# Zhouxunzhe/ManiSkill

Hardware: AMD Instinct MI355X
Metric: env-steps/sec (whole node), PickCube-v1 state-obs 4096 envs/GPU (higher is better)
Workload: dtype f32; 1 GPU; PickCube-v1, Panda, state obs [N,42], pd_joint_delta_pos, num_envs=4096/GPU, sim 100 Hz / control 20 Hz = 5 substeps, 15+1 solver iterations, random actions 2*U-1, no resets inside the timed region; envs_per_gpu=4096, substeps=5, parallelism=env-sharded x1, no collective on the env path, solver_overflow_envs=0

## Files before the change

maniskill_amd/csrc/mssim_solve16.h:

```cpp
#pragma once
#include "mssim_limits.h"

#ifndef S16_WAVES
#define S16_WAVES 4
#endif
#define WSYNC() do { __builtin_amdgcn_fence(__ATOMIC_RELEASE, "wavefront"); __builtin_amdgcn_wave_barrier(); __builtin_amdgcn_fence(__ATOMIC_ACQUIRE, "wavefront"); } while (0)
#define BSYNC() __syncthreads()
#ifndef S16_ENVS_PER_BLOCK
#define S16_ENVS_PER_BLOCK 4
#endif
#define S16_COM_(nr) ((nr) == 4 ? 300 : 0)
#define S16_COM S16_COM_(NR)
#define S16_ANC 8
#define S16_VEC 32
#define S16_PT 96
#define S16_PT_LINK 1
#define S16_PT_FREE 17
#define S16_MAX_FREE S16_MAX_FREE_(NR)
#define S16_PT_KIN_(nr) (S16_PT_FREE + S16_MAX_FREE_(nr))
#define S16_PT_KIN S16_PT_KIN_(NR)
#define S16_MAX_HIT 64
#define S16_BP (S16_PT + 7 * S16_PT_LINK)
#define S16_U_(nr) ((nr) == 4 ? 320 : 272)
#define S16_U S16_U_(NR)
// ... 779 lines not shown
            float r[24];
            const float4* rp = reinterpret_cast<const float4*>(M.shape_pack + 24 * s);
#pragma unroll
            for (int k2 = 0; k2 < 6; k2++) { const float4 t = rp[k2]; r[4 * k2] = t.x; r[4 * k2 + 1] = t.y; r[4 * k2 + 2] = t.z; r[4 * k2 + 3] = t.w; }
            int ty = __float_as_int(r[18]);
            const int slot = __float_as_int(r[21]);
            int hull_first = M.shape_hull[2 * s], hull_count = M.shape_hull[2 * s + 1];
            if (slot < 0) {
              shF[k] = pose_t{f3{r[0], r[1], r[2]}, qnormalized(q4{r[3], r[4], r[5], r[6]})};
              shP[k][0] = r[7]; shP[k][1] = r[8]; shP[k][2] = r[9];
              shBc[k] = f3{r[10], r[11], r[12]};
              shBr[k] = r[13];
              shH[k] = f3{r[14], r[15], r[16]};
            } else {
              shF[k] = pose_soa(M.env_shape_frame, 7 * slot, N, e);
              const float* pp = M.env_shape_param + (size_t)(4 * slot) * N + e;
              const int w0 = __float_as_int(pp[0]);
              ty = w0 & 7;
              shP[k][0] = pp[(size_t)N]; shP[k][1] = pp[2 * (size_t)N]; shP[k][2] = pp[3 * (size_t)N];
              const float* bb = M.env_shape_bound + (size_t)(4 * slot) * N + e;
              shBc[k] = f3{bb[0], bb[(size_t)N], bb[2 * (size_t)N]};
              shBr[k] = bb[3 * (size_t)N];
              shH[k] = (ty == SH_BOX || ty == SH_CONVEX || ty == SH_TRIMESH) ? f3{shP[k][0], shP[k][1], shP[k][2]}
                     : ty == SH_SPHERE ? f3{shP[k][0], shP[k][0], shP[k][0]}
                     : ty == SH_CAPSULE ? f3{shP[k][1] + shP[k][0], shP[k][0], shP[k][0]}
                     : f3{shP[k][1], shP[k][0], shP[k][0]};
              hull_count = (w0 >> 3) & 127; hull_first = w0 >> 10;
            }
            shMu[k] = r[17];
            shTr[k] = r[22];
            shSlot[k] = pose_slot<NR>(__float_as_int(r[19]), __float_as_int(r[20]));
            shPk[k] = (unsigned)ty | ((unsigned)hull_count << 3) | ((unsigned)(shSlot[k] + 1) << 10) | ((unsigned)hull_first << 15);
          }
        }
      }
      EXP_DUP(DUP_SHAPE)
#pragma unroll
      for (int k = 0; k < 2; k++) {
        const int s = cl + GW * k;
        if (s < M.n_shape) {
          pose_t P = pose_t{f3{0, 0, 0}, q4{1, 0, 0, 0}};
          if (shSlot[k] >= 0) P = lds_pose(L + S16_PT + 7 * shSlot[k]);
          const pose_t W = pmul(P, shF[k]);
          const f3 bcw = P.p + qrot(P.q, shBc[k]);
          float* o = L + S16_NP_SHP + S16_SHP * s;
          lds_pose_store(o, W);
          o[7] = shP[k][0]; o[8] = shP[k][1]; o[9] = shP[k][2];
          o[10] = bcw.x; o[11] = bcw.y; o[12] = bcw.z; o[13] = shBr[k];
          o[14] = __uint_as_float(shPk[k]);
          o[15] = shMu[k];
          o[16] = shH[k].x; o[17] = shH[k].y; o[18] = shH[k].z; o[19] = shTr[k];
        }
      }
      WSYNC();
      PH(22);
      int nh = 0;
      int nmesh = 0;
      bool hit_over = false;
      auto cull_round = [&](int p, int sab) __attribute__((always_inline)) {
        bool surv = false;
        const int sa = sab & 0xFF, sb = (sab >> 8) & 0xFF;
        if (sab >= 0) {
          const float* ta_ = L + S16_NP_SHP + S16_SHP * sa;
          const float* tb_ = L + S16_NP_SHP + S16_SHP * sb;
          const int ta = (int)(__float_as_uint(ta_[14]) & 7u);
          const f3 cb = f3{tb_[10], tb_[11], tb_[12]};
          const float ra = ta_[13], rb = tb_[13];
          bool cull;
          if (ta == SH_PLANE) {
            const m3 R = qmat(q4{ta_[3], ta_[4], ta_[5], ta_[6]});
            cull = dot(mcol(R, 0), cb - f3{ta_[0], ta_[1], ta_[2]}) > rb + M.contact_offset;
          } else {
            const f3 d = cb - f3{ta_[10], ta_[11], ta_[12]};
            const float rr = ra + rb + M.contact_offset;
            cull = dot(d, d) > rr * rr;
          }
          const int s1a = (int)((__float_as_uint(ta_[14]) >> 10) & 31u), s1b = (int)((__float_as_uint(tb_[14]) >> 10) & 31u);
          auto inactive = [&](int s1) {
            const int b = s1 - 1 - S16_PT_FREE;
            return s1 == 0 || (b >= 0 && b < S16_MAX_FREE && fw_at(b) <= 0.f);
          };
          const int tb = (int)(__float_as_uint(tb_[14]) & 7u);
          surv = !cull && !(inactive(s1a) && inactive(s1b)) && ta != SH_NONE && tb != SH_NONE;
        }
        const unsigned long long bal = __ballot(surv);
        const unsigned m16 = (unsigned)(bal >> (16 * g)) & 0xFFFFu;
        if (surv) reinterpret_cast<int*>(L)[S16_NP_SCR + nh + __popc(m16 & ((1u << c) - 1u))] = p | (sa << 16) | (sb << 24);
        nh += __popc(m16);
      };
#ifdef EXP_CULL_ROUNDS
      const int n_pair_cull = M.n_pair < 16 * EXP_CULL_ROUNDS ? M.n_pair : 16 * EXP_CULL_ROUNDS;
#else
      const int n_pair_cull = M.n_pair;
#endif
      EXP_DUP(DUP_CULL) {
      if (dup_) { WSYNC(); nh = 0; nmesh = 0; }
      EXP_DUP(DUP_CULL1) {
        if (dup_) { WSYNC(); nh = 0; }
        int sab_next = lead ? M.pair_packed[c] : -1;
#pragma unroll 1
        for (int base = 0; base < n_pair_cull; base += 16) {
          const int sab = sab_next;
          sab_next = lead ? M.pair_packed[base + 16 + c] : -1;
          cull_round(base + c, sab);
        }
      }
      WSYNC();
      const int nh_s1 = nh;
      EXP_DUP(DUP_CULL2) {
        int nh2 = 0;
        if (dup_) { WSYNC(); nmesh = 0; }
#pragma unroll 1
        for (int base = 0; base < nh_s1; base += 16) {
          const int idx = base + c;
          bool keep = false, mesh = false;
          int pk = 0;
          if (idx < nh_s1) {
            pk = reinterpret_cast<const int*>(L)[S16_NP_SCR + idx];
            const float* ta_ = L + S16_NP_SHP + S16_SHP * ((pk >> 16) & 0xFF);
            const float* tb_ = L + S16_NP_SHP + S16_SHP * ((pk >> 24) & 0xFF);
            keep = true;
            if ((int)(__float_as_uint(ta_[14]) & 7u) != SH_PLANE) {
              const m3 RA = qmat(q4{ta_[3], ta_[4], ta_[5], ta_[6]}), RB = qmat(q4{tb_[3], tb_[4], tb_[5], tb_[6]});
              const f3 d = f3{tb_[10], tb_[11], tb_[12]} - f3{ta_[10], ta_[11], ta_[12]};
              keep = !obb_separated(RA, f3{ta_[16], ta_[17], ta_[18]}, RB, f3{tb_[16], tb_[17], tb_[18]}, d, M.contact_offset);
            }
            mesh = TRI && keep && (int)(__float_as_uint(tb_[14]) & 7u) == SH_TRIMESH;
            keep = keep && !mesh;
          }
          if (TRI) {
            const unsigned mm = (unsigned)(__ballot(mesh) >> (16 * g)) & 0xFFFFu;
            const int rankm = nmesh + __popc(mm & ((1u << c) - 1u));
            if (mesh) {
              if (rankm < S16_MAX_HIT) reinterpret_cast<int*>(L)[S16_REC + rankm] = pk;
              else hit_over = true;
            }
            nmesh = min(nmesh + __popc(mm), S16_MAX_HIT);
          }
          const unsigned m16 = (unsigned)(__ballot(keep) >> (16 * g)) & 0xFFFFu;
          const int rank = nh2 + __popc(m16 & ((1u << c) - 1u));
          if (keep) {
            if (rank < S16_MAX_HIT) reinterpret_cast<int*>(L)[S16_NP_HIT + rank] = pk;
            else hit_over = true;
          }
          nh2 += __popc(m16);
        }
        nh = nh2 < S16_MAX_HIT ? nh2 : S16_MAX_HIT;
        if (!live) { nh = 0; nmesh = 0; }
      }
      }
      WSYNC();
      if (__any(hit_over) && hit_over && live) atomicOr(&S.overflow[e], MSSIM_OVERFLOW_HITS);
      PH(23);
      int nml = 0;
      int nbl = 0;
      int npl = 0;
      {
        unsigned char* const ml = reinterpret_cast<unsigned char*>(L + S16_NP_ML);
        unsigned char* const bl = reinterpret_cast<unsigned char*>(L + S16_NP_BL);
        unsigned char* const pll = reinterpret_cast<unsigned char*>(L + S16_NP_PL);
        bool over = false;
        for (int base = 0; base < nh; base += 16) {
          const int idx = base + c;
          bool is_mpr = false, is_bb = false, is_ph = false;
          if (idx < nh) {
            const int pk = reinterpret_cast<const int*>(L)[S16_NP_HIT + idx];
            const int ta = (int)(__float_as_uint(L[S16_NP_SHP + S16_SHP * ((pk >> 16) & 0xFF) + 14]) & 7u);
            const int tb = (int)(__float_as_uint(L[S16_NP_SHP + S16_SHP * ((pk >> 24) & 0xFF) + 14]) & 7u);
            is_bb = ta == SH_BOX && tb == SH_BOX;
            is_ph = ta == SH_PLANE && tb == SH_CONVEX;
            is_mpr = !(ta == SH_PLANE || is_bb || (TRI && tb == SH_TRIMESH));
            reinterpret_cast<int*>(L)[S16_NP_CNT + idx] = 0;
          }
          const unsigned m16 = (unsigned)(__ballot(is_mpr) >> (16 * g)) & 0xFFFFu;
          const int rank = nml + __popc(m16 & ((1u << c) - 1u));
          if (is_mpr) {
            if (rank < S16_MAX_MPR) ml[rank] = (unsigned char)idx;
            else over = true;
          }
          nml += __popc(m16);
          const unsigned b16 = (unsigned)(__ballot(is_bb) >> (16 * g)) & 0xFFFFu;
          if (is_bb) bl[nbl + __popc(b16 & ((1u << c) - 1u))] = (unsigned char)idx;
          nbl += __popc(b16);
          const unsigned p16 = (unsigned)(__ballot(is_ph) >> (16 * g)) & 0xFFFFu;
          if (is_ph) pll[npl + __popc(p16 & ((1u << c) - 1u))] = (unsigned char)idx;
          npl += __popc(p16);
        }
        if (__any(over) && over && live) atomicOr(&S.overflow[e], MSSIM_OVERFLOW_CONVEX);
        nml = nml < S16_MAX_MPR ? nml : S16_MAX_MPR;
      }
      int cum[EPW + 1], mcum[EPW + 1], bcum[EPW + 1];
      cum[0] = mcum[0] = bcum[0] = 0;
#pragma unroll
      for (int j = 0; j < EPW; j++) {
        cum[j + 1] = cum[j] + __shfl(nh, GW * j);
        mcum[j + 1] = mcum[j] + __shfl(nml, GW * j);
        bcum[j + 1] = bcum[j] + __shfl(nbl, GW * j);
      }
      const int T = cum[EPW], TM = mcum[EPW], TB = bcum[EPW];
      const bool bb_lane = NR == 1 && TB > S16_MAX_BBC && T <= 64;
      bool pool_over = false;
      WSYNC();
      PH_ADD(14, (TM + EPW - 1) / EPW);
      (void)mcum;
      PH_ADD(26, T);
      auto pool_alloc = [&](float* Lg, int cnt) __attribute__((always_inline)) -> int {
        int off = atomicAdd(reinterpret_cast<int*>(Lg + S16_NP_ALLOC), cnt);
        if (off + cnt > MSSIM_MAX_RAW_POINTS) { pool_over = true; off = -1; }
        return off;
      };
      for (int t0 = 0; t0 < T; t0 += 64) {
        const int t = t0 + lane64;
        const bool has = t < T;
        int ge = 0;
#pragma unroll
        for (int j = 1; j < EPW; j++) ge += (has && t >= cum[j]) ? 1 : 0;
        const int idx = has ? t - cum[ge] : 0;
        float* Lg = smw + ge * S16_ENV_FLOATS;
        manifold_t m;
        manifold_clear(m);
        bool mine = false;
        if (has) {
          const int pk = reinterpret_cast<const int*>(Lg)[S16_NP_HIT + idx];
          const shape_t A = shape_from_table(M, Lg + S16_NP_SHP + S16_SHP * ((pk >> 16) & 0xFF));
          const shape_t B = shape_from_table(M, Lg + S16_NP_SHP + S16_SHP * ((pk >> 24) & 0xFF));
          PH_ADD(27, __popcll(__ballot(A.type == SH_PLANE)));
          PH_ADD(28, __popcll(__ballot(A.type == SH_BOX && B.type == SH_BOX)));
          PH(10);
          const bool is_plane = A.type == SH_PLANE && B.type != SH_CONVEX, is_bb = bb_lane && A.type == SH_BOX && B.type == SH_BOX;
          if (is_plane) collide_plane(A, B, M.contact_offset, m);
          PH(11);
          if (is_bb) collide_box_box<16>(A, B, M.contact_offset, m, L + S16_NP_SCR + c);
          PH(12);
          mine = is_plane || is_bb;
        }
        WSYNC();
        if (t0 == 0) {
          if (c == 0 && lead) reinterpret_cast<int*>(L)[S16_NP_ALLOC] = 0;
          WSYNC();
        }
        if (mine && m.count > 0) {
          const int off = pool_alloc(Lg, m.count);
          if (off >= 0) {
            reinterpret_cast<int*>(Lg)[S16_NP_CNT + idx] = m.count;
            reinterpret_cast<int*>(Lg)[S16_NP_OFF + idx] = off;
            float* hn = Lg + S16_NP_HN + 3 * idx;
            hn[0] = m.n.x; hn[1] = m.n.y; hn[2] = m.n.z;
#pragma unroll
            for (int k = 0; k < 4; k++)
              if (k < m.count) *reinterpret_cast<float4*>(Lg + S16_NP_POOL + 4 * (off + k)) = float4{m.x[k].x, m.x[k].y, m.x[k].z, m.sep[k]};
          }
        }
      }
      if (T == 0) {
        if (c == 0 && lead) reinterpret_cast<int*>(L)[S16_NP_ALLOC] = 0;
      }
      if (c == 0 && lead) { blk_nml[gb] = nml; blk_nbl[gb] = bb_lane ? 0 : nbl; blk_npl[gb] = npl; }
      BSYNC();
      PH(13);
      BT_T0b;
      {
        int4 hd = int4{-1, 0, 0, 0};
        if (live && nml > 0) hd = *reinterpret_cast<const int4*>(S.pcm + ((size_t)e * MSSIM_PCM_SLOTS + c) * S16_PCM_LEN);
        const int4 hd0 = hd;
        unsigned char* const slot_of = reinterpret_cast<unsigned char*>(L + S16_NP_SLOT);
        const unsigned char* const ml = reinterpret_cast<const unsigned char*>(L + S16_NP_ML);
        auto b16 = [&](bool v) __attribute__((always_inline)) { return (unsigned)(__ballot(v) >> (16 * g)) & 0xFFFFu; };
        for (int k = 0; k < nml; k++) {
          const int idx = ml[k];
          const int p = reinterpret_cast<const int*>(L)[S16_NP_HIT + idx] & 0xFFFF;
          unsigned m16 = b16(hd.x == p);
          bool fresh = false;
          if (m16 == 0u) {
            fresh = true;
            m16 = b16(hd.x < 0);
            if (m16 == 0u) {
              int st = hd.z < pcm_tick ? hd.z : 0x7FFFFFFF;
              int mn = st;
              mn = min(mn, __builtin_amdgcn_update_dpp(0, mn, 0x128, 0xF, 0xF, false));
              mn = min(mn, __builtin_amdgcn_update_dpp(0, mn, 0x124, 0xF, 0xF, false));
              mn = min(mn, __builtin_amdgcn_update_dpp(0, mn, 0x122, 0xF, 0xF, false));
              mn = min(mn, __builtin_amdgcn_update_dpp(0, mn, 0x121, 0xF, 0xF, false));
              m16 = mn != 0x7FFFFFFF ? b16(st == mn) : 0u;
            }
          }
          const int si = m16 ? (__ffs(m16) - 1) : -1;
          if (c == si) {
            if (fresh) { hd.x = p; hd.y = 0; hd.w = 0; }
            hd.z = pcm_tick;
          }
          if (c == 0) slot_of[idx] = si < 0 ? 255 : (unsigned char)(si | (fresh ? 0x80 : 0));
        }
        if (live && (hd.x != hd0.x || hd.y != hd0.y || hd.z != hd0.z || hd.w != hd0.w))
          *reinterpret_cast<int4*>(S.pcm + ((size_t)e * MSSIM_PCM_SLOTS + c) * S16_PCM_LEN) = hd;
      }
      __threadfence_block();
      BSYNC();
      BT_T(17);
      int TMb = 0;
#pragma unroll
      for (int j = 0; j < BLK_ENVS; j++) TMb += blk_nml[j];
      for (int t0 = 0; t0 < TMb; t0 += BLK_GRPS) {
        const bool has = t0 + grp < TMb;
        const int t = has ? t0 + grp : t0;
        int ge = 0, k = t;
#pragma unroll
        for (int j = 0; j < BLK_ENVS - 1; j++) {
          const int nj = blk_nml[j];
          const bool past = ge == j && k >= nj;
          k -= past ? nj : 0;
          ge += past ? 1 : 0;
        }
        float* Lg = sm + ge * S16_ENV_FLOATS;
        const int idx = reinterpret_cast<const unsigned char*>(Lg + S16_NP_ML)[k];
        const int pk = reinterpret_cast<const int*>(Lg)[S16_NP_HIT + idx];
        const shape_t A = shape_from_table(M, Lg + S16_NP_SHP + S16_SHP * ((pk >> 16) & 0xFF));
        const shape_t B = shape_from_table(M, Lg + S16_NP_SHP + S16_SHP * ((pk >> 24) & 0xFF));
        SupCoop16 sup;
        sup.c = c;
        SupCoop16::load_one(sup.va, A, c);
        SupCoop16::load_one(sup.vb, B, c);
        const int sbyte = reinterpret_cast<const unsigned char*>(Lg + S16_NP_SLOT)[idx];
        const bool cached = has && sbyte != 255;
        const bool fresh = cached && (sbyte & 0x80);
        float* const slot = S.pcm + ((size_t)(chunk * BLK_ENVS + ge) * MSSIM_PCM_SLOTS + (cached ? (sbyte & 15) : 0)) * S16_PCM_LEN;
        auto b16 = [&](bool v) __attribute__((always_inline)) { return (unsigned)(__ballot(v) >> (16 * g)) & 0xFFFFu; };
        int npts = 0, grow = 0;
        bool queried_empty = false;
        f3 relp0 = f3{0, 0, 0}, nloc = f3{1, 0, 0};
        float relR0[9] = {1, 0, 0, 0, 1, 0, 0, 0, 1};
        f3 pA = f3{0, 0, 0}, pB = f3{0, 0, 0};
        float s0 = 0.f;
        if (cached && !fresh) {
          const int4 h4 = *reinterpret_cast<const int4*>(slot);
          npts = h4.y; grow = h4.w >> 8; queried_empty = h4.w & 1;
          const float4 r1 = *reinterpret_cast<const float4*>(slot + 4), r2 = *reinterpret_cast<const float4*>(slot + 8), r3 = *reinterpret_cast<const float4*>(slot + 12),
                       r4 = *reinterpret_cast<const float4*>(slot + 16);
          relp0 = f3{r1.x, r1.y, r1.z};
          relR0[0] = r2.x; relR0[1] = r2.y; relR0[2] = r2.z; relR0[3] = r2.w; relR0[4] = r3.x; relR0[5] = r3.y; relR0[6] = r3.z; relR0[7] = r3.w; relR0[8] = r4.x;
          nloc = f3{r4.y, r4.z, r4.w};
          if (c < 4) {
            const float* pp = slot + 20 + 7 * c;
            pA = f3{pp[0], pp[1], pp[2]}; pB = f3{pp[3], pp[4], pp[5]}; s0 = pp[6];
          }
        }
        BT_T(18);
        const float offset = M.contact_offset;
        {
          const f3 nw = mmulv(A.rot, nloc);
          const f3 wA = A.c + mmulv(A.rot, pA), wB = B.c + mmulv(B.rot, pB);
          const f3 d = wA - wB;
          const float dn = dot(d, nw);
          const f3 tt = d - nw * dn;
// ... 472 lines not shown
            }
          } else if (A.type == SH_SPHERE) {
            cand1(0, A.c, A.p0, c == 0);
          } else if (A.type == SH_CAPSULE) {
            const f3 ax = mcol(A.rot, 0) * A.p1;
            cand1(0, c == 0 ? A.c - ax : A.c + ax, A.p0, c < 2);
          } else if (A.type == SH_CONVEX) {
#pragma unroll
            for (int k = 0; k < 4; k++) cand1(k, A.c + mmulv(A.rot, sup.va[k]), 0.f, c + 16 * k < A.nverts);
          } else {
            cand1(0, support(A, -nf), 0.f, c == 0);
          }
          s_low = -gmax16(-s_low);
#pragma unroll
          for (int k = 0; k < 4; k++) ok[k] = ok[k] && Sp[k] <= s_low + MSSIM_TRI_SLACK;
          auto cid = [&](int k) __attribute__((always_inline)) {
            if (A.type == SH_BOX && k >= 1) return c < 11 ? 64 + (c - 8) : 67 + 3 * (c - 11) + (k - 1);
            return c + 16 * k;
          };
          f3 mx[4];
          float msep[4];
          int cnt = 0;
#pragma unroll 1
          for (int r = 0; r < 4; r++) {
            float best = 3e38f;
#pragma unroll
            for (int k = 0; k < 4; k++) best = fminf(best, ok[k] ? Sp[k] : 3e38f);
            best = -gmax16(-best);
            if (!(best < 3e38f)) break;
            int id = 1 << 20;
#pragma unroll
            for (int k = 3; k >= 0; k--) id = (ok[k] && Sp[k] <= best + MSSIM_TRI_TIE) ? min(id, cid(k)) : id;
            id = gmin16i(id);
            const int owner = id >= 67 ? 11 + (id - 67) / 3 : (id >= 64 ? 8 + (id - 64) : (id & 15));
            const int slot = id >= 67 ? 1 + (id - 67) % 3 : (id >= 64 ? 1 : (id >> 4));
            const f3 mine = slot == 0 ? X[0] : (slot == 1 ? X[1] : (slot == 2 ? X[2] : X[3]));
            const f3 px = f3{gbc(mine.x, owner), gbc(mine.y, owner), gbc(mine.z, owner)};
            const float psep = gbc(slot == 0 ? Sp[0] : (slot == 1 ? Sp[1] : (slot == 2 ? Sp[2] : Sp[3])), owner);
#pragma unroll
            for (int t2 = 0; t2 < 4; t2++)
              if (t2 == cnt) { mx[t2] = px; msep[t2] = psep; }
            if (c == owner) {
#pragma unroll
              for (int k = 0; k < 4; k++) ok[k] = ok[k] && k != slot;
            }
            cnt++;
          }
          f3 nrm = nf;
          const bool ask = has && cnt == 0 && s_low < offset;
          if (__any(ask)) {
            f3 inside;
            {
              float w[3];
              closest_on_triangle(q0 - A.c, q1 - A.c, q2 - A.c, w);
              inside = q0 * w[0] + q1 * w[1] + q2 * w[2];
            }
            manifold_t gq;
            manifold_clear(gq);
            if (ask) collide_mpr_t(A, Tr, offset, gq, sup, true, inside);
            if (ask && gq.count > 0 && !(gq.sep[0] < s_low - 1e-3f)) {
              const bool face = dot(nf, gq.n) > 0.5f;
              nrm = face ? nf : gq.n;
              mx[0] = gq.x[0]; msep[0] = gq.sep[0];
              cnt = 1;
              if (face && A.type == SH_BOX) {
                const f3 foot = gq.x[0] - nf * dot(gq.x[0] - q0, nf), dd = foot - q0;
                const float d20 = dot(dd, e0), d21 = dot(dd, e1);
                const float v = (d11 * d20 - d01 * d21) / den, w = (d00 * d21 - d01 * d20) / den;
                float t_in;
                const bool above = box_above(foot, t_in);
                if (v < -tol || w < -tol || v + w > 1.f + tol || !above) cnt = 0;
                mx[0] = foot + nf * (0.5f * t_in); msep[0] = t_in;
              }
            }
          }
          if (has && cnt > 0) {
            int off = 0;
            if (c == 0) off = pool_alloc(Lg, cnt);
            off = gbci(off, 0);
            if (off >= 0) {
              if (c == 0) {
                reinterpret_cast<int*>(Lg)[S16_NP_CNT + idx] = cnt;
                reinterpret_cast<int*>(Lg)[S16_NP_OFF + idx] = off;
                float* hn = Lg + S16_NP_HN + 3 * idx;
                hn[0] = nrm.x; hn[1] = nrm.y; hn[2] = nrm.z;
              }
              if (c < cnt) {
                const f3 x = c == 0 ? mx[0] : (c == 1 ? mx[1] : (c == 2 ? mx[2] : mx[3]));
                const float sp = c == 0 ? msep[0] : (c == 1 ? msep[1] : (c == 2 ? msep[2] : msep[3]));
                *reinterpret_cast<float4*>(Lg + S16_NP_POOL + 4 * (off + c)) = float4{x.x, x.y, x.z, sp};
              }
            }
          }
        }
        BSYNC();
        PH(31);
      }
      BT_T(22);
      PH(25);
      {
        int TBb = 0, TPb = 0;
#pragma unroll
        for (int j = 0; j < BLK_ENVS; j++) { TBb += blk_nbl[j]; TPb += blk_npl[j]; }
#ifdef EXP_NO_STAGE_C
        TBb = 0; TPb = 0;
#endif
        for (int t = grp; t < TBb + TPb; t += BLK_GRPS) {
          const bool ph = t >= TBb;
          int ge = 0, k = ph ? t - TBb : t;
#pragma unroll
          for (int j = 0; j < BLK_ENVS - 1; j++) {
            const int nj = ph ? blk_npl[j] : blk_nbl[j];
            const bool past = ge == j && k >= nj;
            k -= past ? nj : 0;
            ge += past ? 1 : 0;
          }
          float* Lg = sm + ge * S16_ENV_FLOATS;
          const int idx = ph ? reinterpret_cast<const unsigned char*>(Lg + S16_NP_PL)[k] : reinterpret_cast<const unsigned char*>(Lg + S16_NP_BL)[k];
          const int pk = reinterpret_cast<const int*>(Lg)[S16_NP_HIT + idx];
          const shape_t A = shape_from_table(M, Lg + S16_NP_SHP + S16_SHP * ((pk >> 16) & 0xFF));
          const shape_t B = shape_from_table(M, Lg + S16_NP_SHP + S16_SHP * ((pk >> 24) & 0xFF));
          float* const xscr = NR == 4 ? L + S16_XSCR + 44 * (r - 1) : L + S16_NP_KEY;
          float* out = lead ? L + S16_NP_BOUT : xscr + 24;
          if (ph) collide_plane_hull_coop(A, B, M.contact_offset, out, c, g);
          else collide_box_box_coop(A, B, M.contact_offset, lead ? L + S16_NP_BSCR : xscr, out, c, g);
          const int cnt = __float_as_int(out[0]);
          if (cnt > 0) {
            int off = 0;
            if (c == 0) off = pool_alloc(Lg, cnt);
            off = gbci(off, 0);
            if (off >= 0) {
              if (c == 0) {
                reinterpret_cast<int*>(Lg)[S16_NP_CNT + idx] = cnt;
                reinterpret_cast<int*>(Lg)[S16_NP_OFF + idx] = off;
              }
              if (c < 3) Lg[S16_NP_HN + 3 * idx + c] = out[1 + c];
              if (c < cnt) *reinterpret_cast<float4*>(Lg + S16_NP_POOL + 4 * (off + c)) = float4{out[4 + 4 * c], out[5 + 4 * c], out[6 + 4 * c], out[7 + 4 * c]};
            }
          }
        }
      }
      BSYNC();
      (void)bcum; (void)TB;
      if (__any(pool_over) && pool_over && live) atomicOr(&S.overflow[e], MSSIM_OVERFLOW_RAW);
      WSYNC();
      PH(24);
      BT_T0b;
      {
        int* const cnt_ = reinterpret_cast<int*>(L + S16_NP_CNT);
        const int* const off_ = reinterpret_cast<const int*>(L + S16_NP_OFF);
        int* const keep_ = reinterpret_cast<int*>(L + S16_NP_KEEP);
        int* const key_ = reinterpret_cast<int*>(L + S16_NP_KEY);
        const int* const hit_ = reinterpret_cast<const int*>(L + S16_NP_HIT);
        for (int i = c; i < nh; i += 16) {
          const int pk = hit_[i];
          const unsigned pa = __float_as_uint(L[S16_NP_SHP + S16_SHP * ((pk >> 16) & 0xFF) + 14]), pb = __float_as_uint(L[S16_NP_SHP + S16_SHP * ((pk >> 24) & 0xFF) + 14]);
          const bool tors = fmaxf(L[S16_NP_SHP + S16_SHP * ((pk >> 16) & 0xFF) + 19], L[S16_NP_SHP + S16_SHP * ((pk >> 24) & 0xFF) + 19]) > 0.f;
          key_[i] = (int)(((pa >> 10) & 31u) | (((pb >> 10) & 31u) << 8)) | (tors ? 1 << 16 : 0);
        }
        WSYNC();
        {
          unsigned dist = 0u;
          auto free_of = [&](int slot1) { return (slot1 > S16_PT_FREE && slot1 <= S16_PT_FREE + S16_MAX_FREE) ? slot1 - 1 - S16_PT_FREE : -1; };
          auto disturber = [&](int slot1) {
            if (slot1 > S16_PT_LINK && slot1 <= S16_PT_FREE) return true;
            const int b = free_of(slot1);
            return b >= 0 && fw_at(b) > 0.f && !fc_at(b);
          };
          for (int i = c; i < nh; i += 16) {
            if (cnt_[i] <= 0) continue;
            const int ky = key_[i];
            const int s1a = ky & 31, s1b = (ky >> 8) & 31;
            const int ba = free_of(s1a), bb = free_of(s1b);
            if (ba >= 0 && disturber(s1b)) dist |= 1u << ba;
            if (bb >= 0 && disturber(s1a)) dist |= 1u << bb;
          }
          dist |= __shfl_xor(dist, 8, 16); dist |= __shfl_xor(dist, 4, 16); dist |= __shfl_xor(dist, 2, 16); dist |= __shfl_xor(dist, 1, 16);
          if constexpr (NR > 1) dist = (unsigned)env_bci((int)dist, 0);
          fdist = dist;
#pragma unroll
          for (int b = 0; b < S16_MAX_FREE; b++)
            if (b < nf && fwake[b] <= 0.f && ((dist >> b) & 1u)) fwake[b] = MSSIM_WAKE_TIME;
          for (int i = c; i < nh; i += 16) {
            const int ky = key_[i];
            const int ba = free_of(ky & 31), bb = free_of((ky >> 8) & 31);
            const bool sa_ = ba >= 0 && fw_at(ba) <= 0.f, sb_ = bb >= 0 && fw_at(bb) <= 0.f;
            if (sa_ || sb_) cnt_[i] = 0;
          }
          WSYNC();
        }
        BT_T(8);
        bool any_big = false;
        for (int i = c; i < nh; i += 16) {
          int anchor = i;
          const int ci = cnt_[i];
          if (ci > 0) {
            const int ky = key_[i] & 0xFFFF;
            const f3 ni = f3{L[S16_NP_HN + 3 * i], L[S16_NP_HN + 3 * i + 1], L[S16_NP_HN + 3 * i + 2]};
            for (int k = 0; k < i; k++) {
              if (cnt_[k] > 0 && (key_[k] & 0xFFFF) == ky && dot(f3{L[S16_NP_HN + 3 * k], L[S16_NP_HN + 3 * k + 1], L[S16_NP_HN + 3 * k + 2]}, ni) >= MSSIM_PATCH_COS) { anchor = k; break; }
            }
          }
          keep_[i] = (anchor << 4) | ((1 << ci) - 1);
        }
        WSYNC();
        BT_T(25);
        for (int a = c; a < nh; a += 16) {
          if ((keep_[a] >> 4) != a || cnt_[a] == 0) continue;
          int total = 0, tflag = 0;
          for (int i = a; i < nh; i++) {
            const bool mem = (keep_[i] >> 4) == a;
            total += mem ? cnt_[i] : 0;
            tflag |= (mem && cnt_[i] > 0) ? (key_[i] >> 16) & 1 : 0;
          }
          key_[a] |= (tflag << 17) | (total > 4 ? 1 << 18 : 0);
          any_big = any_big || total > 4;
        }
        WSYNC();
        if (__any(any_big)) {
          unsigned short* const cl = reinterpret_cast<unsigned short*>(L + S16_NP_ML);
          auto b16 = [&](bool v) __attribute__((always_inline)) { return (unsigned)(__ballot(v) >> (16 * g)) & 0xFFFFu; };
          for (int a = 0; a < nh; a++) {
            if (!((key_[a] >> 18) & 1)) continue;
            const f3 na = f3{L[S16_NP_HN + 3 * a], L[S16_NP_HN + 3 * a + 1], L[S16_NP_HN + 3 * a + 2]};
            int n = 0;
            for (int base = a; base < nh; base += 16) {
              const int i = base + c;
              const bool mem = i < nh && (keep_[i] >> 4) == a && cnt_[i] > 0;
              const int ni = mem ? cnt_[i] : 0;
              const unsigned b0 = b16(ni & 1), b1 = b16(ni & 2), b2 = b16(ni & 4), lt = (1u << c) - 1u;
              const int pre = n + __popc(b0 & lt) + 2 * __popc(b1 & lt) + 4 * __popc(b2 & lt);
              if (mem) {
                const int of = off_[i];
                for (int q = 0; q < ni; q++)
                  if (pre + q < 64) cl[pre + q] = (unsigned short)((4 * i + q) | ((of + q) << 8));
              }
              n += __popc(b0) + 2 * __popc(b1) + 4 * __popc(b2);
            }
            WSYNC();
            int i0 = -1, i1 = -1, i2 = -1, i3 = -1;
            if (n <= 64) {
              float4 P[4];
              bool has[4];
#pragma unroll
              for (int k = 0; k < 4; k++) {
                has[k] = c + 16 * k < n;
                const int w = has[k] ? cl[c + 16 * k] : 0;
                P[k] = *reinterpret_cast<const float4*>(L + S16_NP_POOL + 4 * (w >> 8));
              }
              auto point_at = [&](int pos) __attribute__((always_inline)) { return *reinterpret_cast<const float4*>(L + S16_NP_POOL + 4 * (cl[pos] >> 8)); };
              auto first_pos = [&](const bool (&ok)[4]) __attribute__((always_inline)) {
                int p = 1 << 20;
#pragma unroll
                for (int k = 3; k >= 0; k--) p = ok[k] ? c + 16 * k : p;
                p = gmin16i(p);
                return p == (1 << 20) ? -1 : p;
              };
              float v[4];
              bool ok[4];
              float best = 3e38f;
#pragma unroll
              for (int k = 0; k < 4; k++) best = fminf(best, has[k] ? P[k].w : 3e38f);
              best = -gmax16(-best);
#pragma unroll
              for (int k = 0; k < 4; k++) ok[k] = has[k] && P[k].w <= best + MSSIM_PATCH_TIE_SEP;
              const int q0 = first_pos(ok);
              {
                int near_ = 0;
#pragma unroll
                for (int k = 0; k < 4; k++) near_ += __popc(b16(has[k] && P[k].w <= best + MSSIM_PATCH_SLACK));
                if (near_ >= 3) {
#pragma unroll
                  for (int k = 0; k < 4; k++) has[k] = has[k] && P[k].w <= best + MSSIM_PATCH_SLACK;
                }
              }
              const float4 P0 = point_at(q0);
              const f3 p0 = f3{P0.x, P0.y, P0.z};
              best = -1.f;
#pragma unroll
              for (int k = 0; k < 4; k++) {
                const f3 d = f3{P[k].x, P[k].y, P[k].z} - p0;
                v[k] = dot(d, d);
                has[k] = has[k] && c + 16 * k != q0;
                best = fmaxf(best, has[k] ? v[k] : -1.f);
              }
              best = gmax16(best);
#pragma unroll
              for (int k = 0; k < 4; k++) ok[k] = has[k] && v[k] >= best - MSSIM_PATCH_TIE_REL * best;
              const int q1 = first_pos(ok);
              const float4 P1 = point_at(q1);
              const f3 ed = f3{P1.x, P1.y, P1.z} - p0;
              best = -1.f;
#pragma unroll
              for (int k = 0; k < 4; k++) {
                v[k] = dot(cross(ed, f3{P[k].x, P[k].y, P[k].z} - p0), na);
                has[k] = has[k] && c + 16 * k != q1;
                best = fmaxf(best, has[k] ? fabsf(v[k]) : -1.f);
              }
              best = gmax16(best);
#pragma unroll
              for (int k = 0; k < 4; k++) ok[k] = has[k] && fabsf(v[k]) >= best - MSSIM_PATCH_TIE_REL * best;
              const int q2 = first_pos(ok);
              const float4 P2 = point_at(q2);
              const float sgn2 = dot(cross(ed, f3{P2.x, P2.y, P2.z} - p0), na);
              best = 0.f;
#pragma unroll
              for (int k = 0; k < 4; k++) {
                v[k] = sgn2 >= 0.f ? -v[k] : v[k];
                has[k] = has[k] && c + 16 * k != q2;
                best = fmaxf(best, has[k] ? v[k] : 0.f);
              }
              best = gmax16(best);
              int q3 = -1;
              if (best > MSSIM_PATCH_TIE_REL * fabsf(sgn2)) {
#pragma unroll
                for (int k = 0; k < 4; k++) ok[k] = has[k] && v[k] >= best - MSSIM_PATCH_TIE_REL * best;
                q3 = first_pos(ok);
              }
              i0 = cl[q0] & 255; i1 = cl[q1] & 255; i2 = cl[q2] & 255; i3 = q3 >= 0 ? (cl[q3] & 255) : -1;
              for (int i = a + c; i < nh; i += 16) {
                if ((keep_[i] >> 4) != a) continue;
                int mk = 0;
                if ((i0 >> 2) == i) mk |= 1 << (i0 & 3);
                if ((i1 >> 2) == i) mk |= 1 << (i1 & 3);
                if ((i2 >> 2) == i) mk |= 1 << (i2 & 3);
                if (i3 >= 0 && (i3 >> 2) == i) mk |= 1 << (i3 & 3);
                keep_[i] = (a << 4) | mk;
              }
            } else if (c == 0) {
          const f3 na = f3{L[S16_NP_HN + 3 * a], L[S16_NP_HN + 3 * a + 1], L[S16_NP_HN + 3 * a + 2]};
              auto scan0 = [&](auto&& f) __attribute__((always_inline)) {
                for (int i = a; i < nh; i++) {
                  if ((keep_[i] >> 4) != a) continue;
                  const int cn = cnt_[i], of = off_[i];
                  for (int q = 0; q < cn; q++) f(4 * i + q, *reinterpret_cast<const float4*>(L + S16_NP_POOL + 4 * (of + q)));
                }
              };
              int i0 = -1, i1 = -1, i2 = -1, i3 = -1;
              float best = 3e38f;
              f3 p0 = f3{0, 0, 0}, p1 = f3{0, 0, 0};
              scan0([&](int, float4 P) { best = fminf(best, P.w); });
              scan0([&](int id, float4 P) { if (i0 < 0 && P.w <= best + MSSIM_PATCH_TIE_SEP) { i0 = id; p0 = f3{P.x, P.y, P.z}; } });
              int near_ = 0;
              const float low = best + MSSIM_PATCH_SLACK;
              scan0([&](int, float4 P) { near_ += P.w <= low ? 1 : 0; });
              const float lim = near_ >= 3 ? low : 3e38f;
              auto scan_all = scan0;
              auto scan = [&](auto&& f) __attribute__((always_inline)) {
                scan_all([&](int id, float4 P) { if (P.w <= lim) f(id, P); });
              };
              best = -1.f;
              scan([&](int id, float4 P) {
                const f3 d = f3{P.x, P.y, P.z} - p0;
                if (id != i0) best = fmaxf(best, dot(d, d));
              });
              scan([&](int id, float4 P) {
                const f3 d = f3{P.x, P.y, P.z} - p0;
                if (i1 < 0 && id != i0 && dot(d, d) >= best - MSSIM_PATCH_TIE_REL * best) { i1 = id; p1 = f3{P.x, P.y, P.z}; }
              });
              const f3 ed = p1 - p0;
              best = -1.f;
              scan([&](int id, float4 P) {
                if (id != i0 && id != i1) best = fmaxf(best, fabsf(dot(cross(ed, f3{P.x, P.y, P.z} - p0), na)));
              });
              float sgn2 = 0.f;
              scan([&](int id, float4 P) {
                const float ar = dot(cross(ed, f3{P.x, P.y, P.z} - p0), na);
                if (i2 < 0 && id != i0 && id != i1 && fabsf(ar) >= best - MSSIM_PATCH_TIE_REL * best) { i2 = id; sgn2 = ar; }
              });
              best = 0.f;
              scan([&](int id, float4 P) {
                const float ar = dot(cross(ed, f3{P.x, P.y, P.z} - p0), na);
                if (id != i0 && id != i1 && id != i2) best = fmaxf(best, sgn2 >= 0.f ? -ar : ar);
              });
              if (best > MSSIM_PATCH_TIE_REL * fabsf(sgn2))
                scan([&](int id, float4 P) {
                  const float ar = dot(cross(ed, f3{P.x, P.y, P.z} - p0), na);
                  const float v = sgn2 >= 0.f ? -ar : ar;
                  if (i3 < 0 && id != i0 && id != i1 && id != i2 && v >= best - MSSIM_PATCH_TIE_REL * best) i3 = id;
                });
              for (int i = a; i < nh; i++) {
                if ((keep_[i] >> 4) != a) continue;
                int mk = 0;
                if ((i0 >> 2) == i) mk |= 1 << (i0 & 3);
                if ((i1 >> 2) == i) mk |= 1 << (i1 & 3);
                if ((i2 >> 2) == i) mk |= 1 << (i2 & 3);
                if (i3 >= 0 && (i3 >> 2) == i) mk |= 1 << (i3 & 3);
                keep_[i] = (a << 4) | mk;
              }

            }
            WSYNC();
          }
        }
        BT_T(23);
        (void)0;
        WSYNC();
        int offs[4] = {0, 0, 0, 0}, offe[4] = {0, 0, 0, 0};
        float trr[4] = {-1.f, -1.f, -1.f, -1.f};
        int tot = 0;
        {
          auto b16 = [&](bool v) __attribute__((always_inline)) { return (unsigned)(__ballot(v) >> (16 * g)) & 0xFFFFu; };
          for (int a = 0; a < nh; a++) {
            if ((keep_[a] >> 4) != a || cnt_[a] == 0) continue;
            const bool tpatch = (key_[a] >> 17) & 1;
            float tr = 0.f;
            for (int base = a & ~15; base < nh; base += 16) {
              const int i = base + c;
              const int wi = i < nh ? keep_[i] : 0;
              const bool mem = i >= a && i < nh && (wi >> 4) == a;
              const int ni = mem ? __popc(wi & 15) : 0;
              const unsigned b0 = b16(ni & 1), b1 = b16(ni & 2), b2 = b16(ni & 4), lt = (1u << c) - 1u;
              const int pre = tot + __popc(b0 & lt) + 2 * __popc(b1 & lt) + 4 * __popc(b2 & lt);
#pragma unroll
              for (int k = 0; k < 4; k++)
                if (mem && (base >> 4) == k) offs[k] = pre;
              tot += __popc(b0) + 2 * __popc(b1) + 4 * __popc(b2);
              if (tpatch) {
                float t = 0.f;
                if (mem && cnt_[i] > 0 && ((key_[i] >> 16) & 1)) {
                  const int pkj = hit_[i];
                  t = fmaxf(L[S16_NP_SHP + S16_SHP * ((pkj >> 16) & 0xFF) + 19], L[S16_NP_SHP + S16_SHP * ((pkj >> 24) & 0xFF) + 19]);
                }
                tr = fmaxf(tr, gmax16(t));
              }
            }
            if (tpatch) {
#pragma unroll
              for (int k = 0; k < 4; k++)
                if (c + 16 * k == a) { offe[k] = tot; trr[k] = tr; }
              tot++;
            }
          }
        }
#pragma unroll
        for (int k = 0; k < 4; k++) {
          const int i = c + 16 * k;
          if (i >= nh) continue;
          const int wi = keep_[i];
          const int mk = wi & 15, a = wi >> 4;
          const bool is_anchor = a == i && cnt_[i] > 0;
          if (mk == 0 && !is_anchor) continue;
          int off = offs[k];
          const int off_end = offe[k];
          const bool my_tors = is_anchor && trr[k] >= 0.f;
          const float my_tr = trr[k];
          const int pk = hit_[i];
          const int sa = (pk >> 16) & 0xFF, sb = (pk >> 24) & 0xFF;
          const float mu = 0.5f * (L[S16_NP_SHP + S16_SHP * sa + 15] + L[S16_NP_SHP + S16_SHP * sb + 15]);
          const int slA = (int)((__float_as_uint(L[S16_NP_SHP + S16_SHP * sa + 14]) >> 10) & 31u) - 1, slB = (int)((__float_as_uint(L[S16_NP_SHP + S16_SHP * sb + 14]) >> 10) & 31u) - 1;
          const int bodies = (int)(slot_lane_mask<NR>(L, slA, n, 0) | (slot_lane_mask<NR>(L, slB, n, 0) << 16));
          const int bodies1 = NR > 1 ? (int)(slot_lane_mask<NR>(L, slA, n, 1) | (slot_lane_mask<NR>(L, slB, n, 1) << 16)) : 0;
          const int bodies2 = NR > 2 ? (int)(slot_lane_mask<NR>(L, slA, n, 2) | (slot_lane_mask<NR>(L, slB, n, 2) << 16)) : 0;
          const int bodies3 = NR > 2 ? (int)(slot_lane_mask<NR>(L, slA, n, 3) | (slot_lane_mask<NR>(L, slB, n, 3) << 16)) : 0;
          const f3 nn = f3{L[S16_NP_HN + 3 * i], L[S16_NP_HN + 3 * i + 1], L[S16_NP_HN + 3 * i + 2]};
          const int of = off_[i];
          for (int q = 0; q < 4; q++) {
            if (!((mk >> q) & 1)) continue;
            if (off < MAXC) {
              const float4 P = *reinterpret_cast<const float4*>(L + S16_NP_POOL + 4 * (of + q));
              float* r = L + S16_REC + S16_REC_LEN * off;
              r[0] = nn.x; r[1] = nn.y; r[2] = nn.z;
              r[3] = P.x; r[4] = P.y; r[5] = P.z;
              r[6] = P.w - M.rest_offset;
              r[7] = __int_as_float((pk & 0xFFFF) | (a << 16) | (q << 24) | ((TRI && (__float_as_uint(L[S16_NP_SHP + S16_SHP * sb + 14]) & 7u) == SH_TRIMESH) ? 1 << 27 : 0));
              r[8] = __int_as_float(bodies);
              r[9] = mu;
              if constexpr (NR > 1) r[10] = __int_as_float(bodies1);
              if constexpr (NR > 2) { r[11] = __int_as_float(bodies2); r[12] = __int_as_float(bodies3); }
            }
            off++;
          }
          if (my_tors && off_end < MAXC) {
            float* r = L + S16_REC + S16_REC_LEN * off_end;
            r[0] = nn.x; r[1] = nn.y; r[2] = nn.z;
            r[3] = 0.f; r[4] = 0.f; r[5] = 0.f; r[6] = 0.f;
            r[7] = __int_as_float((pk & 0xFFFF) | (a << 16) | (1 << 30));
            r[8] = __int_as_float(bodies);
            r[9] = mu * my_tr;
            if constexpr (NR > 1) r[10] = __int_as_float(bodies1);
            if constexpr (NR > 2) { r[11] = __int_as_float(bodies2); r[12] = __int_as_float(bodies3); }
          }
        }
        if (tot > MAXC) { if (live && c == 0) atomicOr(&S.overflow[e], MSSIM_OVERFLOW_CONTACTS); tot = MAXC; }
        nc = tot;
        if constexpr (NR > 1) nc = env_bci(nc, 0);
      }
      WSYNC();
    }
    if (FUSED && last && lead) {
      nold = S.hit_list[e];
#pragma unroll
      for (int k = 0; k < 3; k++)
        if (c + 16 * k < nold) oldp[k] = S.hit_list[(size_t)(1 + c + 16 * k) * N + e];
    }
    BT_T(24);
    PH(21);

    float qt_c = 0.f, qdt_c = 0.f, qf_c = 0.f;
    bool rev_c = false;
    unsigned anc_c = 0u;
    float kp0 = 0.f, kd0 = 0.f, fmax = 3e38f, arm = 0.f, lo_c = -3e38f, hi_c = 3e38f;
    float inert[10] = {0, 0, 0, 0, 0, 0, 0, 0, 0, 0};
    bool grav_c = false, accel_mode = false;
    pose_t JF_c = pose_t{f3{0, 0, 0}, q4{1, 0, 0, 0}};
    f3 al_c = f3{0, 0, 0};
    int par_c = -1;
    if (art) {
      float r[32];
      const float4* rp = reinterpret_cast<const float4*>(M.dof_pack + 32 * c);
#pragma unroll
      for (int k = 0; k < 8; k++) { const float4 t = rp[k]; r[4 * k] = t.x; r[4 * k + 1] = t.y; r[4 * k + 2] = t.z; r[4 * k + 3] = t.w; }
      JF_c = pose_t{f3{r[0], r[1], r[2]}, qnormalized(q4{r[3], r[4], r[5], r[6]})};
      al_c = f3{r[7], r[8], r[9]};
      par_c = __float_as_int(r[10]);
      rev_c = __float_as_int(r[11]) == MSSIM_JOINT_REVOLUTE;
      anc_c = __float_as_uint(r[12]);
      kp0 = r[13]; kd0 = r[14]; fmax = r[15];
      accel_mode = (int)r[16] == MSSIM_DRIVE_ACCELERATION;
      arm = r[17];
      lo_c = r[18]; hi_c = r[19];
#pragma unroll
      for (int k = 0; k < 10; k++) inert[k] = r[20 + k];
      grav_c = __float_as_int(r[30]) != 0;
      qt_c = SOA(S.qt, c); qdt_c = SOA(S.qdt, c); qf_c = SOA(S.qf, c);
    }
    float fin[2][10];
#pragma unroll
    for (int b = 0; b < 2; b++) {
#pragma unroll
      for (int k = 0; k < 10; k++) fin[b][k] = 0.f;
      if (b < nfr) free_inertial_of(M, N, fb0 + b, e, fin[b]);
    }

    const pose_t root = lds_pose(L + S16_PT);
    pose_t bp_c = root;
    f3 aw_c = f3{0, 0, 0}, an_c = f3{0, 0, 0};
    if (art) {
      bp_c = lds_pose(L + S16_BP + 7 * c);
      pose_t Wp0 = root;
      if (par_c >= 0) Wp0 = lds_pose(L + S16_BP + 7 * par_c);
      const pose_t Jw0 = pmul(Wp0, JF_c);
      aw_c = qrot(Jw0.q, al_c);
      an_c = Jw0.p;
    }
    sv6 S_c = sv6{f3{0, 0, 0}, f3{0, 0, 0}};
    if (art) S_c = rev_c ? sv6{aw_c, cross(an_c - O, aw_c)} : sv6{f3{0, 0, 0}, aw_c};
    if (lead) {
      float* p = L + S16_S + 6 * c;
      p[0] = S_c.w.x; p[1] = S_c.w.y; p[2] = S_c.w.z; p[3] = S_c.v.x; p[4] = S_c.v.y; p[5] = S_c.v.z;
      L[S16_VEC + c] = qd_c;
    }
    WSYNC();
    sv6 V = sv6{f3{0, 0, 0}, f3{0, 0, 0}};
    for (int i = 0; i < n; i++) {
      float m = (((anc_c | self_c) >> i) & 1u) ? L[S16_VEC + i] : 0.f;
      const float* p = L + S16_S + 6 * i;
      V.w += f3{p[0], p[1], p[2]} * m;
      V.v += f3{p[3], p[4], p[5]} * m;
    }
    if (lead) {
      sv6 T = crossm(V, S_c);
      float* p = L + S16_T + 6 * c;
      p[0] = T.w.x * qd_c; p[1] = T.w.y * qd_c; p[2] = T.w.z * qd_c; p[3] = T.v.x * qd_c; p[4] = T.v.y * qd_c; p[5] = T.v.z * qd_c;
    }
    WSYNC();
    sv6 Ab = sv6{f3{0, 0, 0}, f3{0, 0, 0}};
    for (int i = 0; i < n; i++) {
      float m = (((anc_c | self_c) >> i) & 1u) ? 1.f : 0.f;
      const float* p = L + S16_T + 6 * i;
      Ab.w += f3{p[0], p[1], p[2]} * m;
      Ab.v += f3{p[3], p[4], p[5]} * m;
    }
    si10 I_c = si10{0.f, f3{0, 0, 0}, s3{0, 0, 0, 0, 0, 0}};
    sf6 Fb_c = sf6{f3{0, 0, 0}, f3{0, 0, 0}};
    if (art) {
      m3 R = qmat(bp_c.q);
      s3 Iw = srotate(R, s3{inert[4], inert[5], inert[6], inert[7], inert[8], inert[9]});
      f3 cm = bp_c.p + mmulv(R, f3{inert[1], inert[2], inert[3]}) - O;
      float m = inert[0], cc = dot(cm, cm);
      Iw.xx += m * (cc - cm.x * cm.x); Iw.yy += m * (cc - cm.y * cm.y); Iw.zz += m * (cc - cm.z * cm.z);
      Iw.xy -= m * cm.x * cm.y; Iw.xz -= m * cm.x * cm.z; Iw.yz -= m * cm.y * cm.z;
      I_c = si10{m, cm * m, Iw};
      sf6 f1 = imul(I_c, Ab);
      sf6 f2 = crossf(V, imul(I_c, V));
      Fb_c = sf6{f1.n + f2.n, f1.f + f2.f};
      if (grav_c) { Fb_c.f -= g3 * m; Fb_c.n -= cross(I_c.h, g3); }
    }
    if (lead) {
      float* p = L + S16_F + 6 * c;
      p[0] = Fb_c.n.x; p[1] = Fb_c.n.y; p[2] = Fb_c.n.z; p[3] = Fb_c.f.x; p[4] = Fb_c.f.y; p[5] = Fb_c.f.z;
      float* qI = L + S16_IC + 10 * c;
      qI[0] = I_c.m; qI[1] = I_c.h.x; qI[2] = I_c.h.y; qI[3] = I_c.h.z;
      qI[4] = I_c.I.xx; qI[5] = I_c.I.yy; qI[6] = I_c.I.zz; qI[7] = I_c.I.xy; qI[8] = I_c.I.xz; qI[9] = I_c.I.yz;
// ... 632 lines not shown
```

Measured before the change: 9.692 million env-steps/s.

## Cull sleeping-body hit pairs before narrowphase and keep contact metadata in registers

Adds an early pass after broadphase that drops cheap hit pairs (plane or box-box) touching sleeping free bodies that no awake body disturbs, so narrowphase no longer computes contacts that would later be zeroed. Counts of the dropped pairs are carried so the box-box lane heuristic still sees the original totals. The contact patch stage also changes: per-hit key, count and keep values stay in registers, wave-level OR and sum reductions use DPP in place of shuffles, and anchor iteration goes over ballot masks instead of serial LDS scans. This removes LDS round trips and barriers, but the culling must exactly match the later sleep test or contacts could be lost.

```diff
diff --git a/maniskill_amd/csrc/mssim_solve16.h b/maniskill_amd/csrc/mssim_solve16.h
--- a/maniskill_amd/csrc/mssim_solve16.h
+++ b/maniskill_amd/csrc/mssim_solve16.h
@@ -955,6 +955,69 @@
       WSYNC();
       if (__any(hit_over) && hit_over && live) atomicOr(&S.overflow[e], MSSIM_OVERFLOW_HITS);
       PH(23);
+      auto free_of = [&](int slot1) { return (slot1 > S16_PT_FREE && slot1 <= S16_PT_FREE + S16_MAX_FREE) ? slot1 - 1 - S16_PT_FREE : -1; };
+      auto disturber = [&](int slot1) {
+        if (slot1 > S16_PT_LINK && slot1 <= S16_PT_FREE) return true;
+        const int b = free_of(slot1);
+        return b >= 0 && fw_at(b) > 0.f && !fc_at(b);
+      };
+      int nh_doomed = 0, nbl_doomed = 0;
+      {
+        bool any_asleep = false;
+#pragma unroll
+        for (int b = 0; b < S16_MAX_FREE; b++) any_asleep = any_asleep || (b < nf && fwake[b] <= 0.f);
+        if (__any(any_asleep && nh > 0)) {
+          int* const hit_ = reinterpret_cast<int*>(L + S16_NP_HIT);
+          auto b16 = [&](bool v) __attribute__((always_inline)) { return (unsigned)(__ballot(v) >> (16 * g)) & 0xFFFFu; };
+          int hk[4];
+          unsigned zz[4];
+          bool light[4], bb_[4];
+          unsigned touch = 0u;
+#pragma unroll
+          for (int k = 0; k < 4; k++) {
+            const int i = c + 16 * k;
+            hk[k] = 0; zz[k] = 0u; light[k] = false; bb_[k] = false;
+            if (i < nh) {
+              const int pk = hit_[i];
+              const unsigned pa = __float_as_uint(L[S16_NP_SHP + S16_SHP * ((pk >> 16) & 0xFF) + 14]), pb = __float_as_uint(L[S16_NP_SHP + S16_SHP * ((pk >> 24) & 0xFF) + 14]);
+              const int s1a = (int)((pa >> 10) & 31u), s1b = (int)((pb >> 10) & 31u);
+              const int ta = (int)(pa & 7u), tb = (int)(pb & 7u);
+              const int ba = free_of(s1a), bb = free_of(s1b);
+              if (ba >= 0 && fw_at(ba) <= 0.f) { zz[k] |= 1u << ba; if (disturber(s1b)) touch |= 1u << ba; }
+              if (bb >= 0 && fw_at(bb) <= 0.f) { zz[k] |= 1u << bb; if (disturber(s1a)) touch |= 1u << bb; }
+              hk[k] = pk;
+              bb_[k] = ta == SH_BOX && tb == SH_BOX;
+              light[k] = bb_[k] || (ta == SH_PLANE && tb != SH_TRIMESH);
+            }
+          }
+          touch |= (unsigned)__builtin_amdgcn_update_dpp(0, (int)touch, 0x128, 0xF, 0xF, false);
+          touch |= (unsigned)__builtin_amdgcn_update_dpp(0, (int)touch, 0x124, 0xF, 0xF, false);
+          touch |= (unsigned)__builtin_amdgcn_update_dpp(0, (int)touch, 0x122, 0xF, 0xF, false);
+          touch |= (unsigned)__builtin_amdgcn_update_dpp(0, (int)touch, 0x121, 0xF, 0xF, false);
+          bool doomed[4];
+          bool any_doomed = false;
+#pragma unroll
+          for (int k = 0; k < 4; k++) {
+            doomed[k] = light[k] && (zz[k] & ~touch) != 0u;
+            any_doomed = any_doomed || doomed[k];
+          }
+          if (__any(any_doomed)) {
+            WSYNC();
+            int w = 0;
+#pragma unroll
+            for (int k = 0; k < 4; k++) {
+              const bool stay = c + 16 * k < nh && !doomed[k];
+              const unsigned m16 = b16(stay);
+              if (stay) hit_[w + __popc(m16 & ((1u << c) - 1u))] = hk[k];
+              w += __popc(m16);
+              nbl_doomed += __popc(b16(doomed[k] && bb_[k]));
+            }
+            nh_doomed = nh - w;
+            nh = w;
+            WSYNC();
+          }
+        }
+      }
       int nml = 0;
       int nbl = 0;
       int npl = 0;
@@ -1000,8 +1063,16 @@
         mcum[j + 1] = mcum[j] + __shfl(nml, GW * j);
         bcum[j + 1] = bcum[j] + __shfl(nbl, GW * j);
       }
-      const int T = cum[EPW], TM = mcum[EPW], TB = bcum[EPW];
-      const bool bb_lane = NR == 1 && TB > S16_MAX_BBC && T <= 64;
+      const int T = cum[EPW], TM = mcum[EPW];
+      int T_all = T, TB = bcum[EPW];
+      if (nf > 0) {
+#pragma unroll
+        for (int j = 0; j < EPW; j++) {
+          T_all += __shfl(nh_doomed, GW * j);
+          TB += __shfl(nbl_doomed, GW * j);
+        }
+      }
+      const bool bb_lane = NR == 1 && TB > S16_MAX_BBC && T_all <= 64;
       bool pool_over = false;
       WSYNC();
       PH_ADD(14, (TM + EPW - 1) / EPW);
@@ -1780,45 +1851,59 @@
         int* const keep_ = reinterpret_cast<int*>(L + S16_NP_KEEP);
         int* const key_ = reinterpret_cast<int*>(L + S16_NP_KEY);
         const int* const hit_ = reinterpret_cast<const int*>(L + S16_NP_HIT);
-        for (int i = c; i < nh; i += 16) {
-          const int pk = hit_[i];
-          const unsigned pa = __float_as_uint(L[S16_NP_SHP + S16_SHP * ((pk >> 16) & 0xFF) + 14]), pb = __float_as_uint(L[S16_NP_SHP + S16_SHP * ((pk >> 24) & 0xFF) + 14]);
-          const bool tors = fmaxf(L[S16_NP_SHP + S16_SHP * ((pk >> 16) & 0xFF) + 19], L[S16_NP_SHP + S16_SHP * ((pk >> 24) & 0xFF) + 19]) > 0.f;
-          key_[i] = (int)(((pa >> 10) & 31u) | (((pb >> 10) & 31u) << 8)) | (tors ? 1 << 16 : 0);
-        }
-        WSYNC();
-        {
+        auto b16 = [&](bool v) __attribute__((always_inline)) { return (unsigned)(__ballot(v) >> (16 * g)) & 0xFFFFu; };
+        auto b64 = [&](const bool (&v)[4]) __attribute__((always_inline)) {
+          return (unsigned long long)(b16(v[0]) | (b16(v[1]) << 16)) | ((unsigned long long)(b16(v[2]) | (b16(v[3]) << 16)) << 32);
+        };
+        int kyr[4], cnr[4], kpr[4];
+        bool touches_free = false;
+#pragma unroll
+        for (int k = 0; k < 4; k++) {
+          const int i = c + 16 * k;
+          kyr[k] = 0; cnr[k] = 0; kpr[k] = 0;
+          if (i < nh) {
+            const int pk = hit_[i];
+            const unsigned pa = __float_as_uint(L[S16_NP_SHP + S16_SHP * ((pk >> 16) & 0xFF) + 14]), pb = __float_as_uint(L[S16_NP_SHP + S16_SHP * ((pk >> 24) & 0xFF) + 14]);
+            const bool tors = fmaxf(L[S16_NP_SHP + S16_SHP * ((pk >> 16) & 0xFF) + 19], L[S16_NP_SHP + S16_SHP * ((pk >> 24) & 0xFF) + 19]) > 0.f;
+            kyr[k] = (int)(((pa >> 10) & 31u) | (((pb >> 10) & 31u) << 8)) | (tors ? 1 << 16 : 0);
+            key_[i] = kyr[k];
+            cnr[k] = cnt_[i];
+            touches_free = touches_free || free_of((int)((pa >> 10) & 31u)) >= 0 || free_of((int)((pb >> 10) & 31u)) >= 0;
+          }
+        }
+        fdist = 0u;
+        if (nf > 0 && __any(touches_free)) {
           unsigned dist = 0u;
-          auto free_of = [&](int slot1) { return (slot1 > S16_PT_FREE && slot1 <= S16_PT_FREE + S16_MAX_FREE) ? slot1 - 1 - S16_PT_FREE : -1; };
-          auto disturber = [&](int slot1) {
-            if (slot1 > S16_PT_LINK && slot1 <= S16_PT_FREE) return true;
-            const int b = free_of(slot1);
-            return b >= 0 && fw_at(b) > 0.f && !fc_at(b);
-          };
-          for (int i = c; i < nh; i += 16) {
-            if (cnt_[i] <= 0) continue;
-            const int ky = key_[i];
-            const int s1a = ky & 31, s1b = (ky >> 8) & 31;
+#pragma unroll
+          for (int k = 0; k < 4; k++) {
+            if (cnr[k] <= 0) continue;
+            const int s1a = kyr[k] & 31, s1b = (kyr[k] >> 8) & 31;
             const int ba = free_of(s1a), bb = free_of(s1b);
             if (ba >= 0 && disturber(s1b)) dist |= 1u << ba;
             if (bb >= 0 && disturber(s1a)) dist |= 1u << bb;
           }
-          dist |= __shfl_xor(dist, 8, 16); dist |= __shfl_xor(dist, 4, 16); dist |= __shfl_xor(dist, 2, 16); dist |= __shfl_xor(dist, 1, 16);
+          dist |= (unsigned)__builtin_amdgcn_update_dpp(0, (int)dist, 0x128, 0xF, 0xF, false);
+          dist |= (unsigned)__builtin_amdgcn_update_dpp(0, (int)dist, 0x124, 0xF, 0xF, false);
+          dist |= (unsigned)__builtin_amdgcn_update_dpp(0, (int)dist, 0x122, 0xF, 0xF, false);
+          dist |= (unsigned)__builtin_amdgcn_update_dpp(0, (int)dist, 0x121, 0xF, 0xF, false);
           if constexpr (NR > 1) dist = (unsigned)env_bci((int)dist, 0);
           fdist = dist;
 #pragma unroll
           for (int b = 0; b < S16_MAX_FREE; b++)
             if (b < nf && fwake[b] <= 0.f && ((dist >> b) & 1u)) fwake[b] = MSSIM_WAKE_TIME;
-          for (int i = c; i < nh; i += 16) {
-            const int ky = key_[i];
-            const int ba = free_of(ky & 31), bb = free_of((ky >> 8) & 31);
+#pragma unroll
+          for (int k = 0; k < 4; k++) {
+            const int i = c + 16 * k;
+            if (i >= nh) continue;
+            const int ba = free_of(kyr[k] & 31), bb = free_of((kyr[k] >> 8) & 31);
             const bool sa_ = ba >= 0 && fw_at(ba) <= 0.f, sb_ = bb >= 0 && fw_at(bb) <= 0.f;
-            if (sa_ || sb_) cnt_[i] = 0;
-          }
-          WSYNC();
-        }
+            if (sa_ || sb_) { cnr[k] = 0; cnt_[i] = 0; }
+          }
+        }
+        WSYNC();
         BT_T(8);
-        bool any_big = false;
+        int anc[4];
+        bool hasp[4];
         for (int i = c; i < nh; i += 16) {
           int anchor = i;
           const int ci = cnt_[i];
@@ -1831,25 +1916,36 @@
           }
           keep_[i] = (anchor << 4) | ((1 << ci) - 1);
         }
+#pragma unroll
+        for (int k = 0; k < 4; k++) {
+          const int i = c + 16 * k;
+          hasp[k] = cnr[k] > 0;
+          kpr[k] = i < nh ? keep_[i] : i << 4;
+          anc[k] = kpr[k] >> 4;
+        }
         WSYNC();
         BT_T(25);
-        for (int a = c; a < nh; a += 16) {
-          if ((keep_[a] >> 4) != a || cnt_[a] == 0) continue;
-          int total = 0, tflag = 0;
-          for (int i = a; i < nh; i++) {
-            const bool mem = (keep_[i] >> 4) == a;
-            total += mem ? cnt_[i] : 0;
-            tflag |= (mem && cnt_[i] > 0) ? (key_[i] >> 16) & 1 : 0;
-          }
-          key_[a] |= (tflag << 17) | (total > 4 ? 1 << 18 : 0);
-          any_big = any_big || total > 4;
-        }
-        WSYNC();
-        if (__any(any_big)) {
+        bool isanc[4];
+#pragma unroll
+        for (int k = 0; k < 4; k++) isanc[k] = hasp[k] && anc[k] == c + 16 * k;
+        const unsigned long long amask = b64(isanc);
+        unsigned long long tmask = 0ull, bmask = 0ull;
+        for (unsigned long long m = amask; m; m &= m - 1ull) {
+          const int a = __ffsll(m) - 1;
+          int t = 0;
+#pragma unroll
+          for (int k = 0; k < 4; k++) t += (hasp[k] && anc[k] == a) ? cnr[k] + (((kyr[k] >> 16) & 1) << 16) : 0;
+          t += __builtin_amdgcn_update_dpp(0, t, 0x128, 0xF, 0xF, false);
+          t += __builtin_amdgcn_update_dpp(0, t, 0x124, 0xF, 0xF, false);
+          t += __builtin_amdgcn_update_dpp(0, t, 0x122, 0xF, 0xF, false);
+          t += __builtin_amdgcn_update_dpp(0, t, 0x121, 0xF, 0xF, false);
+          if ((t >> 16) != 0) tmask |= 1ull << a;
+          if ((t & 0xFFFF) > 4) bmask |= 1ull << a;
+        }
+        if (__any(bmask != 0ull)) {
           unsigned short* const cl = reinterpret_cast<unsigned short*>(L + S16_NP_ML);
-          auto b16 = [&](bool v) __attribute__((always_inline)) { return (unsigned)(__ballot(v) >> (16 * g)) & 0xFFFFu; };
-          for (int a = 0; a < nh; a++) {
-            if (!((key_[a] >> 18) & 1)) continue;
+          for (unsigned long long bm = bmask; bm; bm &= bm - 1ull) {
+            const int a = __ffsll(bm) - 1;
             const f3 na = f3{L[S16_NP_HN + 3 * a], L[S16_NP_HN + 3 * a + 1], L[S16_NP_HN + 3 * a + 2]};
             int n = 0;
             for (int base = a; base < nh; base += 16) {
@@ -2024,29 +2120,33 @@
         BT_T(23);
         (void)0;
         WSYNC();
+        if (bmask != 0ull) {
+#pragma unroll
+          for (int k = 0; k < 4; k++)
+            if (c + 16 * k < nh) kpr[k] = keep_[c + 16 * k];
+        }
         int offs[4] = {0, 0, 0, 0}, offe[4] = {0, 0, 0, 0};
         float trr[4] = {-1.f, -1.f, -1.f, -1.f};
         int tot = 0;
         {
-          auto b16 = [&](bool v) __attribute__((always_inline)) { return (unsigned)(__ballot(v) >> (16 * g)) & 0xFFFFu; };
-          for (int a = 0; a < nh; a++) {
-            if ((keep_[a] >> 4) != a || cnt_[a] == 0) continue;
-            const bool tpatch = (key_[a] >> 17) & 1;
+          for (unsigned long long m = amask; m; m &= m - 1ull) {
+            const int a = __ffsll(m) - 1;
+            const bool tpatch = (tmask >> a) & 1ull;
             float tr = 0.f;
-            for (int base = a & ~15; base < nh; base += 16) {
-              const int i = base + c;
-              const int wi = i < nh ? keep_[i] : 0;
+#pragma unroll
+            for (int k = 0; k < 4; k++) {
+              if (16 * k + 15 < a || 16 * k >= nh) continue;
+              const int i = 16 * k + c;
+              const int wi = kpr[k];
               const bool mem = i >= a && i < nh && (wi >> 4) == a;
               const int ni = mem ? __popc(wi & 15) : 0;
               const unsigned b0 = b16(ni & 1), b1 = b16(ni & 2), b2 = b16(ni & 4), lt = (1u << c) - 1u;
               const int pre = tot + __popc(b0 & lt) + 2 * __popc(b1 & lt) + 4 * __popc(b2 & lt);
-#pragma unroll
-              for (int k = 0; k < 4; k++)
-                if (mem && (base >> 4) == k) offs[k] = pre;
+              if (mem) offs[k] = pre;
               tot += __popc(b0) + 2 * __popc(b1) + 4 * __popc(b2);
               if (tpatch) {
                 float t = 0.f;
-                if (mem && cnt_[i] > 0 && ((key_[i] >> 16) & 1)) {
+                if (mem && cnr[k] > 0 && ((kyr[k] >> 16) & 1)) {
                   const int pkj = hit_[i];
                   t = fmaxf(L[S16_NP_SHP + S16_SHP * ((pkj >> 16) & 0xFF) + 19], L[S16_NP_SHP + S16_SHP * ((pkj >> 24) & 0xFF) + 19]);
                 }
@@ -2065,9 +2165,9 @@
         for (int k = 0; k < 4; k++) {
           const int i = c + 16 * k;
           if (i >= nh) continue;
-          const int wi = keep_[i];
+          const int wi = kpr[k];
           const int mk = wi & 15, a = wi >> 4;
-          const bool is_anchor = a == i && cnt_[i] > 0;
+          const bool is_anchor = a == i && cnr[k] > 0;
           if (mk == 0 && !is_anchor) continue;
           int off = offs[k];
           const int off_end = offe[k];
```

New measurement: 10.34 million env-steps/s (median of 6 runs). 1.07x the previous value.
